# YQChen8/SSF-SLAM

Hardware: AMD Instinct MI355X
Metric: LiDAR front-end frames/sec (mask+feature+GN), 64-beam 120k pts, 1/2/4/8 GPUs (higher is better)
Workload: dtype f32 features / f64 mask+solve

## Files before the change

### ssf-slam_amd/csrc/mask_pose.hip

```cpp
#include "ssf_device.hpp"
#include "ssf_internal.hpp"
#include "svd3.hpp"

#include <float.h>
#include <type_traits>

namespace ssf {

#ifndef SSF_MASK_THREADS
#define SSF_MASK_THREADS 768
#endif
constexpr int kMaskThreads = SSF_MASK_THREADS;

#ifdef SSF_MASK_STAMPS
#define SSF_STAMP(slot)                                                                   \
    do {                                                                                  \
        if (threadIdx.x == 0) {                                                           \
            const unsigned long long _t = __builtin_amdgcn_s_memtime();                   \
            out[26 + (slot)] = (double)(_t - stamp0);                                     \
        }                                                                                 \
    } while (0)
#else
#define SSF_STAMP(slot) do { } while (0)
#endif
constexpr int kNW = kMaskThreads / 64;
#ifndef SSF_LLOYD_DEEP
#define SSF_LLOYD_DEEP 2
#endif
constexpr int kLloydDeep = SSF_LLOYD_DEEP;
#ifndef SSF_KPP_DEEP
#define SSF_KPP_DEEP 2
#endif
constexpr int kKppBlocks = 4096;
constexpr double kPi = 3.14159265358979323846;
#ifndef SSF_LLOYD_FULL_PASSES
#define SSF_LLOYD_FULL_PASSES 4
#endif
constexpr int kLloydFullPasses = SSF_LLOYD_FULL_PASSES;
#ifndef SSF_LLOYD_REFULL
#define SSF_LLOYD_REFULL 4
#endif
constexpr int kLloydRefull = SSF_LLOYD_REFULL;
#ifndef SSF_LLOYD_REC_DEEP
#define SSF_LLOYD_REC_DEEP 8
#endif
constexpr int kLloydRecDeep = SSF_LLOYD_REC_DEEP;
constexpr int kLQ = SSF_LLOYD_REC_DEEP * 128;
constexpr int kLloydMax = 300;

SSF_DEV constexpr int up(int i, int j) { return i * 6 - (i * (i - 1)) / 2 + (j - i); }

struct MaskShared {
    double mean[6], tol;
    double tot[28];
    double cen[12], csn[2], cenp[12], csnp[2];
    double x0[6], ktot[16];
    double mu[12], U[42], logdet[2], logw[2];
    double Aq[21], bq[6], cq, C0;
    double rand1, rand2;
    double lb;
    double C[36], L[36], Li[36];
    double sums[29];
    double lsum[14];
    double lhist[kLloydMax * 9];
    float lb1[512], lb2[512];
    int64_t c0, c1;
    double dg_cyc, dg_n, dg_lab, dg_wfull, dg_full1;
#ifdef SSF_MASK_STAMPS
    double dg_e[3];
#endif
    double passes;
    int km_iter, em_iter, strict, converged, done, status, label0, bg, bg_pred, lfull;
    double hnk[2], hq[2], hpm[12];
    int hrc[2];
};

template <class T>
SSF_DEV void load_x(const T* __restrict__ P, const T* __restrict__ Fl, int64_t i, double x[6]) {
    x[0] = (double)Fl[3 * i]; x[1] = (double)Fl[3 * i + 1]; x[2] = (double)Fl[3 * i + 2];
    x[3] = (double)P[3 * i];  x[4] = (double)P[3 * i + 1];  x[5] = (double)P[3 * i + 2];
}



SSF_DEV int prec_chol6_r(const double (&C)[36], double (&U)[21], double& logdet) {
    double L[36], Li[36];
#pragma unroll
    for (int k = 0; k < 36; ++k) { L[k] = 0.0; Li[k] = 0.0; }
    bool ok = true;
#pragma unroll
    for (int j = 0; j < 6; ++j) {
        double s = C[j * 6 + j];
#pragma unroll
        for (int k = 0; k < j; ++k) s -= L[j * 6 + k] * L[j * 6 + k];
        ok = ok && (s > 0.0);
        L[j * 6 + j] = sqrt(s);
#pragma unroll
        for (int i = j + 1; i < 6; ++i) {
            double v = C[i * 6 + j];
#pragma unroll
            for (int k = 0; k < j; ++k) v -= L[i * 6 + k] * L[j * 6 + k];
            L[i * 6 + j] = v / L[j * 6 + j];
        }
    }
#pragma unroll
    for (int c = 0; c < 6; ++c)
#pragma unroll
        for (int i = c; i < 6; ++i) {
            double v = (i == c) ? 1.0 : 0.0;
#pragma unroll
            for (int k = c; k < i; ++k) v -= L[i * 6 + k] * Li[k * 6 + c];
            Li[i * 6 + c] = v / L[i * 6 + i];
        }
    double ld = 0.0;
#pragma unroll
    for (int i = 0; i < 6; ++i)
#pragma unroll
        for (int j = i; j < 6; ++j) U[up(i, j)] = Li[j * 6 + i];
#pragma unroll
    for (int i = 0; i < 6; ++i) ld += log(Li[i * 6 + i]);
    logdet = ld;
    return ok ? 0 : -1;
}

__device__ __noinline__ int gmm_params2(MaskShared& S, const double* comp1, int init, int64_t n) {
    const int k = (int)(threadIdx.x & 1u);
    const double eps10 = 10.0 * DBL_EPSILON;
    double a[28];
#pragma unroll
    for (int i = 0; i < 28; ++i) a[i] = k == 1 ? comp1[i] : S.tot[i] - comp1[i];
    const double nk = a[0] + eps10;
    double d[6];
#pragma unroll
    for (int i = 0; i < 6; ++i) {
        const double mu = (a[0] * S.mean[i] + a[1 + i]) / nk;
        d[i] = mu - S.mean[i];
        S.hpm[6 * k + i] = mu;
    }
    double C[36];
#pragma unroll
    for (int i = 0; i < 6; ++i)
#pragma unroll
        for (int j = i; j < 6; ++j) {
            double v = a[7 + up(i, j)] - a[1 + i] * d[j] - d[i] * a[1 + j] + a[0] * d[i] * d[j];
            v = v / nk;
            C[i * 6 + j] = v; C[j * 6 + i] = v;
        }
#pragma unroll
    for (int i = 0; i < 6; ++i) C[i * 6 + i] += 1e-6;
    double U[21], ld;
    const int rc = prec_chol6_r(C, U, ld);
    double P[36];
#pragma unroll
    for (int r = 0; r < 6; ++r)
#pragma unroll
        for (int c = r; c < 6; ++c) {
            double v = 0.0;
#pragma unroll
            for (int j = c; j < 6; ++j) v += U[up(r, j)] * U[up(c, j)];
            P[r * 6 + c] = v; P[c * 6 + r] = v;
        }
    double q = 0.0, Pm[6];
#pragma unroll
    for (int r = 0; r < 6; ++r) {
        double v = 0.0;
#pragma unroll
        for (int c = 0; c < 6; ++c) v += P[r * 6 + c] * d[c];
        Pm[r] = v;
        q += d[r] * v;
    }
    S.hnk[k] = nk; S.hq[k] = q; S.hrc[k] = rc;
    __builtin_amdgcn_wave_barrier();
    const bool ok = S.hrc[0] == 0 && S.hrc[1] == 0;
    if (ok) {
#pragma unroll
        for (int i = 0; i < 6; ++i) S.mu[6 * k + i] = S.hpm[6 * k + i];
#pragma unroll
        for (int i = 0; i < 21; ++i) S.U[21 * k + i] = U[i];
        S.logdet[k] = ld;
        double* Pk = k ? S.L : S.C;
#pragma unroll
        for (int i = 0; i < 36; ++i) Pk[i] = P[i];
#pragma unroll
        for (int i = 0; i < 6; ++i) S.hpm[6 * k + i] = Pm[i];
    }
    __builtin_amdgcn_wave_barrier();
    if (k != 0) return 0;
    if (!ok) return -1;
    const double nk0 = S.hnk[0], nk1 = S.hnk[1];
    double w0, w1;
    if (init) { w0 = nk0 / (double)n; w1 = nk1 / (double)n; }
    else { const double sw = nk0 + nk1; w0 = nk0 / sw; w1 = nk1 / sw; }
    S.logw[0] = log(w0); S.logw[1] = log(w1);
    const double* P0 = S.C;
    const double* P1 = S.L;
#pragma unroll
    for (int r = 0; r < 6; ++r) {
#pragma unroll
        for (int c = r; c < 6; ++c) {
            const double A = -0.5 * (P1[r * 6 + c] - P0[r * 6 + c]);
            S.Aq[up(r, c)] = r == c ? A : 2.0 * A;
        }
        S.bq[r] = S.hpm[6 + r] - S.hpm[r];
    }
    S.cq = -0.5 * (S.hq[1] - S.hq[0]) + (S.logdet[1] + S.logw[1]) - (S.logdet[0] + S.logw[0]);
    const double N = S.tot[0];
    double tr = 0.0, lin = 0.0;
#pragma unroll
    for (int r = 0; r < 6; ++r) {
// ... 199 lines not shown
                tt = 1 - m[0][0] + m[1][1] - m[2][2];
                w = m[2][0] - m[0][2]; x = m[0][1] + m[1][0]; y = tt; z = m[1][2] + m[2][1];
            }
        } else {
            if (m[0][0] < -m[1][1]) {
                tt = 1 - m[0][0] - m[1][1] + m[2][2];
                w = m[0][1] - m[1][0]; x = m[2][0] + m[0][2]; y = m[1][2] + m[2][1]; z = tt;
            } else {
                tt = 1 + m[0][0] + m[1][1] + m[2][2];
                w = tt; x = m[1][2] - m[2][1]; y = m[2][0] - m[0][2]; z = m[0][1] - m[1][0];
            }
        }
        const double f = 0.5 / sqrt(tt);
        q[0] = x * f; q[1] = y * f; q[2] = z * f; q[3] = w * f;
    } else if (status == 0) {
        status = SSF_POSE_NOT_ORTHOGONAL;
    }
    for (int i = 0; i < 3; ++i) out[SSF_POSE_OUT_T + i] = t[i];
    for (int i = 0; i < 4; ++i) out[SSF_POSE_OUT_Q + i] = q[i];
    for (int i = 0; i < 9; ++i) out[SSF_POSE_OUT_R + i] = R[i];
    out[SSF_POSE_OUT_NBG] = n;
    return status;
}

constexpr int kSlot = 32;
constexpr int kMaxSplit = kMaskMaxSplit;
constexpr uint32_t kSpinLimit = 1u << 24;
constexpr int kMaxExchanges = 1 + 3 + 300 + 1 + 100 + 1;

struct Split {
    int G, g;
    int64_t r0, r1;
    double* part;
    uint32_t* arrive;
    uint32_t* fail;
    uint32_t seq;
};


SSF_DEV bool wait_arrivals(const Split& X, uint32_t target) {
    uint32_t spins = 0;
    while (__hip_atomic_load(X.arrive, __ATOMIC_RELAXED, __HIP_MEMORY_SCOPE_AGENT) < target) {
        __builtin_amdgcn_s_sleep(2);
        if (++spins > kSpinLimit ||
            __hip_atomic_load(X.fail, __ATOMIC_RELAXED, __HIP_MEMORY_SCOPE_AGENT) != 0u)
            return false;
    }
    return true;
}

template <int N, bool kMin = false>
SSF_DEV bool exchange(Split& X, double (&v)[N], double* tmp, int* okflag) {
    static_assert(N <= kSlot, "exchange: N <= kSlot");
    if (X.G == 1) return true;
    if (X.seq >= (uint32_t)kMaxExchanges) return false;
    double* slot = X.part + (size_t)X.seq * (size_t)X.G * kSlot;
#pragma unroll
    for (int k = 0; k < N; ++k)
        if (threadIdx.x == (unsigned)k)
            __hip_atomic_store(reinterpret_cast<unsigned long long*>(slot + X.g * kSlot + k),
                               (unsigned long long)__double_as_longlong(v[k]), __ATOMIC_RELAXED,
                               __HIP_MEMORY_SCOPE_AGENT);
    X.seq += 1u;
    if (threadIdx.x < 64) {
        asm volatile("s_waitcnt vmcnt(0)" ::: "memory");
        if (threadIdx.x == 0) {
            __builtin_amdgcn_fence(__ATOMIC_RELEASE, "agent");
            asm volatile("s_waitcnt vmcnt(0)" ::: "memory");
            __hip_atomic_fetch_add(X.arrive, 1u, __ATOMIC_RELAXED, __HIP_MEMORY_SCOPE_AGENT);
            const int ok = wait_arrivals(X, (uint32_t)X.G * X.seq) ? 1 : 0;
            __builtin_amdgcn_fence(__ATOMIC_ACQUIRE, "agent");
            asm volatile("s_waitcnt vmcnt(0)" ::: "memory");
            *okflag = ok;
        }
    }
    __syncthreads();
    __builtin_amdgcn_fence(__ATOMIC_ACQUIRE, "wavefront");
    if (!*okflag) return false;
    for (int t = threadIdx.x; t < X.G * N; t += blockDim.x) {
        const int gg = t / N, k = t - gg * N;
        tmp[kSlot + t] = __longlong_as_double((long long)__hip_atomic_load(
            reinterpret_cast<unsigned long long*>(slot + gg * kSlot + k), __ATOMIC_RELAXED,
            __HIP_MEMORY_SCOPE_AGENT));
    }
    __syncthreads();
    if (threadIdx.x < (unsigned)N) {
        double acc = kMin ? __builtin_inf() : 0.0;
        for (int gg = 0; gg < X.G; ++gg) {
            const double x = tmp[kSlot + gg * N + threadIdx.x];
            acc = kMin ? (x < acc ? x : acc) : acc + x;
        }
        tmp[threadIdx.x] = acc;
    }
    __syncthreads();
#pragma unroll
    for (int k = 0; k < N; ++k) v[k] = tmp[k];
    __syncthreads();
    return true;
}

SSF_DEV bool exchange_prefix(Split& X, double v, double* tmp, int* okflag, double& before, double& total) {
    if (X.seq >= (uint32_t)kMaxExchanges) return false;
    double* slot = X.part + (size_t)X.seq * (size_t)X.G * kSlot;
    if (threadIdx.x == 0)
        __hip_atomic_store(reinterpret_cast<unsigned long long*>(slot + X.g * kSlot),
                           (unsigned long long)__double_as_longlong(v), __ATOMIC_RELAXED, __HIP_MEMORY_SCOPE_AGENT);
    X.seq += 1u;
    if (threadIdx.x < 64) {
        asm volatile("s_waitcnt vmcnt(0)" ::: "memory");
        if (threadIdx.x == 0) {
            __builtin_amdgcn_fence(__ATOMIC_RELEASE, "agent");
            asm volatile("s_waitcnt vmcnt(0)" ::: "memory");
            __hip_atomic_fetch_add(X.arrive, 1u, __ATOMIC_RELAXED, __HIP_MEMORY_SCOPE_AGENT);
            const int ok = wait_arrivals(X, (uint32_t)X.G * X.seq) ? 1 : 0;
            __builtin_amdgcn_fence(__ATOMIC_ACQUIRE, "agent");
            asm volatile("s_waitcnt vmcnt(0)" ::: "memory");
            *okflag = ok;
        }
    }
    __syncthreads();
    __builtin_amdgcn_fence(__ATOMIC_ACQUIRE, "wavefront");
    if (!*okflag) return false;
    if (threadIdx.x < (unsigned)X.G)
        tmp[kSlot + threadIdx.x] = __longlong_as_double((long long)__hip_atomic_load(
            reinterpret_cast<unsigned long long*>(slot + threadIdx.x * kSlot), __ATOMIC_RELAXED,
            __HIP_MEMORY_SCOPE_AGENT));
    __syncthreads();
    if (threadIdx.x == 0) {
        double b = 0.0, t = 0.0;
        for (int gg = 0; gg < X.G; ++gg) {
            const double x = tmp[kSlot + gg];
            if (gg < X.g) b += x;
            t += x;
        }
        tmp[0] = b; tmp[1] = t;
    }
    __syncthreads();
    before = tmp[0];
    total = tmp[1];
    __syncthreads();
    return true;
}

SSF_DEV void accum_kabsch(double (&k)[16], const double* x, const double cs[3], const double cd[3]) {
    double s[3], d[3];
    for (int i = 0; i < 3; ++i) { d[i] = x[3 + i] - cd[i]; s[i] = (x[3 + i] + x[i]) - cs[i]; }
    k[0] += 1.0;
#pragma unroll
    for (int i = 0; i < 3; ++i) { k[1 + i] += s[i]; k[4 + i] += d[i]; }
#pragma unroll
    for (int r = 0; r < 3; ++r)
#pragma unroll
        for (int c = 0; c < 3; ++c) k[7 + r * 3 + c] += s[r] * d[c];
}

template <class T>
__global__ __launch_bounds__(kMaskThreads) void k_mask_pose(
    const T* __restrict__ pts, const T* __restrict__ flow,
    const int64_t* __restrict__ frame_off, int mode, const uint8_t* __restrict__ mask_in,
    const double* __restrict__ draws, uint2* __restrict__ lloyd_rec, int reflection,
    uint8_t* __restrict__ bg_mask, double* __restrict__ out_all, int n_frames, int G,
    uint32_t* __restrict__ sync, double* __restrict__ parts, const int32_t* __restrict__ order,
    int tickets) {
    __shared__ MaskShared S;
    __shared__ double red[kNW * 32];
    __shared__ int ired[kNW];
    __shared__ unsigned long long cand_lds[2];
    __shared__ double bsum[kKppBlocks];
    __shared__ uint32_t lq[kNW * kLQ];
    __shared__ double xtmp[kSlot + kMaxSplit * kSlot];
    __shared__ int tk, okflag;
    const int tid = threadIdx.x;
    for (int iter = 0;; ++iter) {
    int f, g = 0;
    if (G == 1 && !tickets) {
        if (iter > 0) break;
        f = blockIdx.x;
    } else {
        __syncthreads();
        if (tid == 0) tk = (int)atomicAdd(sync, 1u);
        __syncthreads();
        f = tk / G;
        g = tk - f * G;
        if (f >= n_frames) break;
    }
    if (order) {
        f = order[f];
        if ((unsigned)f >= (unsigned)n_frames) continue;
    }
    [&]() {
    const int64_t fb = frame_off[f], n = frame_off[f + 1] - fb;
    const T* P = pts + 3 * fb;
    const T* Fl = flow + 3 * fb;
    double* out = out_all + (int64_t)f * SSF_POSE_OUT_STRIDE;
    Split X;
    X.G = G; X.g = g;
    {
        const int64_t chunk = ((n + G - 1) / G + 127) / 128 * 128;
        X.r0 = min(n, (int64_t)g * chunk);
        X.r1 = min(n, X.r0 + chunk);
    }
    X.part = parts + (size_t)f * kMaxExchanges * (size_t)G * kSlot;
    X.arrive = sync + 4 + f;
    X.fail = sync + 4 + n_frames + f;
    X.seq = 0;
    const int64_t r0 = X.r0, r1 = X.r1;
    auto sync_failed = [&]() {
        if (tid == 0) {
            __hip_atomic_store(X.fail, 1u, __ATOMIC_RELAXED, __HIP_MEMORY_SCOPE_AGENT);
            if (g == 0) {
                for (int i = 0; i < SSF_POSE_OUT_STRIDE; ++i) out[i] = 0.0;
                out[SSF_POSE_OUT_STATUS] = SSF_POSE_SYNC_FAILED;
            }
        }
    };
    if (tid == 0) {
        S.passes = 0; S.status = 0; S.km_iter = 0; S.em_iter = 0; S.converged = 0;
        if (g == 0) for (int i = 26; i < SSF_POSE_OUT_STRIDE; ++i) out[i] = 0.0;
    }
#ifdef SSF_MASK_STAMPS
    const unsigned long long stamp0 = __builtin_amdgcn_s_memtime();
#endif
    __syncthreads();

    if (mode != SSF_MASK_GMM) {
        double cs[3] = {0, 0, 0}, cd[3] = {0, 0, 0};
        if (n > 0) {
            double x0[6];
            load_x(P, Fl, 0, x0);
            for (int i = 0; i < 3; ++i) { cd[i] = x0[3 + i]; cs[i] = x0[3 + i] + x0[i]; }
        }
        double k[16];
        for (int i = 0; i < 16; ++i) k[i] = 0.0;
        for (int64_t i = tid; i < n; i += blockDim.x) {
            const uint8_t mv = mask_in[fb + i];
            const bool bg = (mode == SSF_MASK_GT) ? (mv == 0) : (mv != 0);
            if (bg_mask) bg_mask[fb + i] = bg ? 1 : 0;
            if (!bg) continue;
            double x[6];
            load_x(P, Fl, i, x);
            accum_kabsch(k, x, cs, cd);
        }
        block_sum_rs<16>(k, red);
        if (tid == 0) {
            for (int i = 0; i < SSF_POSE_OUT_STRIDE; ++i) out[i] = 0.0;
            for (int i = 0; i < 16; ++i) S.sums[i] = k[i];
            const int st = kabsch_finish(S.sums, cs, cd, reflection, out);
            out[SSF_POSE_OUT_STATUS] = st;
            out[SSF_POSE_OUT_BGLABEL] = -1;
            out[SSF_POSE_OUT_PASSES] = 1;
        }
        return;
    }

    if (n < 2) {
        if (tid == 0 && g == 0) {
            for (int i = 0; i < SSF_POSE_OUT_STRIDE; ++i) out[i] = 0.0;
            out[SSF_POSE_OUT_STATUS] = SSF_POSE_GMM_FAILED;
        }
        return;
    }

    {
        double x0[6];
        load_x(P, Fl, 0, x0);
        double a[27];
#pragma unroll
        for (int i = 0; i < 27; ++i) a[i] = 0.0;
        for_points_deep<kLloydDeep>(P, Fl, r0, r1, [&](int64_t, const double* x, bool val) {
            double v[6], vw[6];
#pragma unroll
            for (int d = 0; d < 6; ++d) { v[d] = x[d] - x0[d]; vw[d] = val ? v[d] : 0.0; a[d] += vw[d]; }
#pragma unroll
            for (int r = 0; r < 6; ++r)
#pragma unroll
                for (int c = r; c < 6; ++c) a[6 + up(r, c)] += vw[r] * v[c];
        });
        block_sum_rs<27>(a, red);
        if (!exchange<27>(X, a, xtmp, &okflag)) { sync_failed(); return; }
        if (tid == 0) {
            const double nn = (double)n;
            double m[6];
            double tol = 0.0;
            for (int d = 0; d < 6; ++d) { m[d] = a[d] / nn; S.mean[d] = x0[d] + m[d]; }
            S.tot[0] = nn;
            for (int d = 0; d < 6; ++d) S.tot[1 + d] = a[d] - nn * m[d];
            for (int r = 0; r < 6; ++r)
                for (int c = r; c < 6; ++c) S.tot[7 + up(r, c)] = a[6 + up(r, c)] - nn * m[r] * m[c];
            for (int d = 0; d < 6; ++d) tol += S.tot[7 + up(d, d)] / nn;
            S.tol = tol / 6.0 * 1e-4;
            for (int d = 0; d < 6; ++d) S.x0[d] = x0[d];
            S.ktot[0] = nn;
            for (int r = 0; r < 3; ++r) { S.ktot[1 + r] = a[r] + a[3 + r]; S.ktot[4 + r] = a[3 + r]; }
            for (int r = 0; r < 3; ++r)
                for (int c = 0; c < 3; ++c) {
                    const int fr = r, pr = 3 + r, pc = 3 + c;
                    const double sfp = a[6 + (fr <= pc ? up(fr, pc) : up(pc, fr))];
                    const double spp = a[6 + (pr <= pc ? up(pr, pc) : up(pc, pr))];
                    S.ktot[7 + r * 3 + c] = sfp + spp;
                }
            S.c0 = (int64_t)draws[3 * f];
            if (S.c0 < 0) S.c0 = 0;
            if (S.c0 >= n) S.c0 = n - 1;
            S.passes = 1;
        }
        __syncthreads();
    }
    SSF_STAMP(0);
    double mean[6];
#pragma unroll
    for (int d = 0; d < 6; ++d) mean[d] = uni(S.mean[d]);

    {
        double c0[6], cn0 = 0.0;
        {
            double x[6];
            load_x(P, Fl, S.c0, x);
            for (int d = 0; d < 6; ++d) { c0[d] = x[d] - mean[d]; cn0 += c0[d] * c0[d]; }
        }
        const int nw = blockDim.x >> 6, w = tid >> 6, lane = lane_id();
        const int64_t nloc = r1 - r0;
        const int64_t seg = (((nloc + nw - 1) / nw) + 63) / 64 * 64;
        const int64_t ws = r0 + (int64_t)w * seg, we = ws + seg < r1 ? ws + seg : r1;
        auto dist0x = [&](const double* x) {
            double dt = 0.0, xs = 0.0;
#pragma unroll
            for (int d = 0; d < 6; ++d) { const double v = x[d] - mean[d]; dt += c0[d] * v; xs += v * v; }
            const double v = (-2.0 * dt + cn0) + xs;
            return v > 0.0 ? v : 0.0;
        };
        auto dist0 = [&](int64_t i) {
            double x[6];
            load_x(P, Fl, i, x);
            return dist0x(x);
        };
        constexpr int kKppDeep = SSF_KPP_DEEP;
        const int64_t wlast = we > ws ? we - 1 : ws;
        const int64_t spw = seg / 64;
        const bool use_blocks = spw * nw <= kKppBlocks;
        double wsum = 0.0;
        T kb[kKppDeep][6];
        if (ws < we) {
#pragma unroll
            for (int k = 0; k < kKppDeep; ++k) load_raw(P, Fl, min(ws + 64 * k + lane, wlast), kb[k]);
        }
        for (int64_t b0 = ws; b0 < we; b0 += 64 * kKppDeep)
#pragma unroll
        for (int k = 0; k < kKppDeep; ++k) {
            const int64_t b = b0 + 64 * k;
            if (b >= we) break;
            const int64_t i = b + lane;
            double x[6];
#pragma unroll
            for (int d = 0; d < 6; ++d) x[d] = (double)kb[k][d];
            load_raw(P, Fl, min(i + 64 * kKppDeep, wlast), kb[k]);
            const double d = i < we ? dist0x(x) : 0.0;
            wsum += d;
            if (use_blocks) {
                double v = d;
#pragma unroll
                for (int o = 1; o < 64; o <<= 1) {
                    const double y = __shfl_up(v, o, 64);
                    if (lane >= o) v += y;
                }
                if (lane == 63) bsum[w * spw + (b - ws) / 64] = v;
            }
        }
        wsum = wave_sum(wsum);
        if (lane == 0) red[w] = wsum;
        if (tid == 0) { cand_lds[0] = (unsigned long long)n; cand_lds[1] = (unsigned long long)n; }
        __syncthreads();
        double pot = 0.0, carry = 0.0;
        for (int k = 0; k < nw; ++k) { if (k == w) carry = pot; pot += red[k]; }
        if (G > 1) {
            double before = 0.0, total = 0.0;
            if (!exchange_prefix(X, pot, xtmp, &okflag, before, total)) { sync_failed(); return; }
            carry += before;
            pot = total;
        }
        if (tid == 0) {
            S.rand1 = draws[3 * f + 1] * pot;
            S.rand2 = draws[3 * f + 2] * pot;
            S.passes += 1;
        }
        const double r1 = draws[3 * f + 1] * pot, r2 = draws[3 * f + 2] * pot;
        const double wtot = red[w];
        bool f1 = carry + wtot < r1 * (1.0 - 1e-9), f2 = carry + wtot < r2 * (1.0 - 1e-9);
        if (use_blocks) {
            int64_t blk1 = -1, blk2 = -1;
            double cb1 = 0.0, cb2 = 0.0;
            if (lane == 0 && !(f1 && f2)) {
                double cr = carry;
                for (int64_t k = 0; ws + 64 * k < we; ++k) {
                    const double tot = bsum[w * spw + k];
                    if (!f1 && blk1 < 0 && cr + tot >= r1) { blk1 = k; cb1 = cr; }
                    if (!f2 && blk2 < 0 && cr + tot >= r2) { blk2 = k; cb2 = cr; }
                    if ((f1 || blk1 >= 0) && (f2 || blk2 >= 0)) break;
                    cr += tot;
                }
            }
            blk1 = __shfl(blk1, 0, 64); blk2 = __shfl(blk2, 0, 64);
            cb1 = __shfl(cb1, 0, 64); cb2 = __shfl(cb2, 0, 64);
#pragma unroll
            for (int j = 0; j < 2; ++j) {
                const int64_t blk = j ? blk2 : blk1;
                if (blk < 0) continue;
                const int64_t b = ws + 64 * blk;
                const int64_t i = b + lane;
                double v = i < we ? dist0(i) : 0.0;
#pragma unroll
                for (int o = 1; o < 64; o <<= 1) {
                    const double y = __shfl_up(v, o, 64);
                    if (lane >= o) v += y;
                }
                const double incl = (j ? cb2 : cb1) + v;
                const uint64_t mm = __ballot(i < we && incl >= (j ? r2 : r1));
                if (mm && lane == 0) atomicMin(&cand_lds[j], (unsigned long long)(b + __ffsll((unsigned long long)mm) - 1));
            }
            f1 = f2 = true;
        }
        for (int64_t b = ws; b < we && !(f1 && f2); b += 64) {
            const int64_t i = b + lane;
            double v = i < we ? dist0(i) : 0.0;
#pragma unroll
            for (int o = 1; o < 64; o <<= 1) {
                const double y = __shfl_up(v, o, 64);
                if (lane >= o) v += y;
            }
            const double incl = carry + v;
            const uint64_t m1 = __ballot(i < we && incl >= r1), m2 = __ballot(i < we && incl >= r2);
            if (!f1 && m1) { f1 = true; if (lane == 0) atomicMin(&cand_lds[0], (unsigned long long)(b + __ffsll((unsigned long long)m1) - 1)); }
            if (!f2 && m2) { f2 = true; if (lane == 0) atomicMin(&cand_lds[1], (unsigned long long)(b + __ffsll((unsigned long long)m2) - 1)); }
            carry += __shfl(v, 63, 64);
        }
        __syncthreads();
        double cmin[2] = {(double)cand_lds[0], (double)cand_lds[1]};
        if (!exchange<2, true>(X, cmin, xtmp, &okflag)) { sync_failed(); return; }
        const int64_t cand[2] = {cmin[0] < (double)n ? (int64_t)cmin[0] : n - 1,
                                 cmin[1] < (double)n ? (int64_t)cmin[1] : n - 1};
        double cc[2][6], ccn[2] = {0.0, 0.0};
        for (int j = 0; j < 2; ++j) {
            double x[6];
            load_x(P, Fl, cand[j], x);
            for (int d = 0; d < 6; ++d) { cc[j][d] = x[d] - mean[d]; ccn[j] += cc[j][d] * cc[j][d]; }
        }
        double cp[2] = {0.0, 0.0};
        if (ws < we) {
#pragma unroll
            for (int k = 0; k < kKppDeep; ++k) load_raw(P, Fl, min(ws + 64 * k + lane, wlast), kb[k]);
        }
        for (int64_t b0 = ws; b0 < we; b0 += 64 * kKppDeep)
#pragma unroll
        for (int k = 0; k < kKppDeep; ++k) {
            const int64_t b = b0 + 64 * k;
            if (b >= we) break;
            const int64_t i = b + lane;
            double x[6];
#pragma unroll
            for (int d = 0; d < 6; ++d) x[d] = (double)kb[k][d];
            load_raw(P, Fl, min(i + 64 * kKppDeep, wlast), kb[k]);
            if (i < we) {
                double xs = 0.0, dt0 = 0.0, dt1 = 0.0, dtc = 0.0;
#pragma unroll
                for (int d = 0; d < 6; ++d) {
                    const double v = x[d] - mean[d];
                    dtc += c0[d] * v; xs += v * v; dt0 += cc[0][d] * v; dt1 += cc[1][d] * v;
                }
                double di = (-2.0 * dtc + cn0) + xs;
                di = di > 0.0 ? di : 0.0;
                double v0 = (-2.0 * dt0 + ccn[0]) + xs, v1 = (-2.0 * dt1 + ccn[1]) + xs;
                v0 = v0 > 0.0 ? v0 : 0.0; v1 = v1 > 0.0 ? v1 : 0.0;
                cp[0] += v0 < di ? v0 : di;
                cp[1] += v1 < di ? v1 : di;
            }
        }
        block_sum<2>(cp, red);
        if (!exchange<2>(X, cp, xtmp, &okflag)) { sync_failed(); return; }
        if (tid == 0) {
            const int best = cp[1] < cp[0] ? 1 : 0;
            S.c1 = cand[best];
            for (int d = 0; d < 6; ++d) { S.cen[d] = c0[d]; S.cen[6 + d] = cc[best][d]; }
            for (int d = 0; d < 12; ++d) S.cenp[d] = 0.0;
            S.csnp[0] = S.csnp[1] = 0.0;
            S.passes += 2;
        }
        __syncthreads();
    }

    SSF_STAMP(1);
    if (tid == 0) { S.strict = 0; S.done = 0; S.lfull = 1; S.dg_cyc = S.dg_n = S.dg_lab = S.dg_wfull = S.dg_full1 = 0.0; }
    uint2* __restrict__ LR = lloyd_rec + ((fb + 2 * (int64_t)f + 1) & ~(int64_t)1);
    uint32_t* __restrict__ LQ =
        reinterpret_cast<uint32_t*>(lloyd_rec + frame_off[n_frames] + 2 * (int64_t)n_frames + 2) + fb +
        64 * (int64_t)f;
    for (int it = 0; it < kLloydMax; ++it) {
        if (tid == 0) {
            double* h = S.lhist + 9 * it;
            for (int k = 0; k < 2; ++k) {
                double sn = 0.0;
                for (int d = 0; d < 6; ++d) sn += S.cen[6 * k + d] * S.cen[6 * k + d];
                S.csn[k] = sn;
            }
            for (int d = 0; d < 6; ++d) h[d] = S.cen[6 + d] - S.cen[d];
            h[6] = S.csn[0] - S.csn[1];
            h[7] = sqrt(S.csn[0]) + sqrt(S.csn[1]);
            h[8] = S.csn[0] + S.csn[1];
        }
        __syncthreads();
        if (tid < it) {
            const double* h = S.lhist + 9 * it;
            const double* g = S.lhist + 9 * tid;
            double dw = 0.0;
            for (int d = 0; d < 6; ++d) dw += (h[d] - g[d]) * (h[d] - g[d]);
            S.lb1[tid] = __double2float_ru(2.0 * sqrt(dw) + 2e-13 * (h[7] + g[7]));
            S.lb2[tid] = __double2float_ru(fabs(h[6] - g[6]) + 1e-13 * (h[8] + g[8]));
        }
        __syncthreads();
        const double csn0 = uni(S.csn[0]), csn1 = uni(S.csn[1]);
        double acc[14];
#pragma unroll
        for (int k = 0; k < 14; ++k) acc[k] = 0.0;
        int changed = 0, nlab = 0;
        const bool full = S.lfull != 0;
#ifdef SSF_MASK_STAMPS
        const unsigned long long pass_t0 = __builtin_amdgcn_s_memtime();
#endif
        const bool wrec = it >= kLloydFullPasses - 1;
        auto label = [&](auto wrec_c, int64_t i, const double* x, int lp, bool val) {
            const LdsDouble* cen = lds_laundered(S.cen);
            double v[6], dt0 = 0.0, dt1 = 0.0, vn = 0.0;
#pragma unroll
            for (int d = 0; d < 6; ++d) {
                v[d] = x[d] - mean[d];
                dt0 += v[d] * cen[d]; dt1 += v[d] * cen[6 + d]; vn += v[d] * v[d];
            }
            const double D0 = -2.0 * dt0 + csn0, D1 = -2.0 * dt1 + csn1;
            const int l = D1 < D0 ? 1 : 0;
            double d1 = full ? (double)l : (double)(l - lp), d0 = full ? 1.0 - d1 : -d1;
            d1 = val ? d1 : 0.0; d0 = val ? d0 : 0.0;
            changed += val && (it == 0 || l != lp);
            acc[0] += d0; acc[7] += d1;
#pragma unroll
            for (int d = 0; d < 6; ++d) { acc[1 + d] += d0 * v[d]; acc[8 + d] += d1 * v[d]; }
            const uint32_t gb = __float_as_uint((float)fabs(D0 - D1));
            const uint32_t nvb = (__float_as_uint(__builtin_sqrtf((float)vn)) + 4u + 0x1FFu) & 0x7FFFFE00u;
            if constexpr (decltype(wrec_c)::value) LR[val ? i : n] = make_uint2(gb ? gb - 1u : 0u, nvb | (uint32_t)it | ((uint32_t)l << 31));
        };
        if (full) {
            const double cpn0 = uni(S.csnp[0]), cpn1 = uni(S.csnp[1]);
            auto full_pass = [&](auto wrec_c) {
                for_points_deep<kLloydDeep>(P, Fl, r0, r1, [&](int64_t i, const double* x, bool val) {
                    const LdsDouble* cenp = lds_laundered(S.cenp);
                    double dp0 = 0.0, dp1 = 0.0;
#pragma unroll
                    for (int d = 0; d < 6; ++d) {
                        const double v = x[d] - mean[d];
                        dp0 += v * cenp[d]; dp1 += v * cenp[6 + d];
                    }
                    const int lp = (-2.0 * dp1 + cpn1) < (-2.0 * dp0 + cpn0) ? 1 : 0;
                    label(wrec_c, i, x, lp, val);
                });
            };
            if (wrec) full_pass(std::true_type{});
            else full_pass(std::false_type{});
            nlab = (int)((r1 - r0 - tid + blockDim.x - 1) / blockDim.x);
        } else {
            const int w = __builtin_amdgcn_readfirstlane(tid >> 6), lane = lane_id();
            const int64_t seg = ((r1 - r0 + kNW - 1) / kNW + 127) / 128 * 128;
            const int64_t ws = r0 + (int64_t)w * seg, we = ws + seg < r1 ? ws + seg : r1;
            uint32_t* __restrict__ WQ = LQ + ws;
            const int64_t qspare = n - ws;
            const uint4* __restrict__ LR4 = reinterpret_cast<const uint4*>(LR);
            const int64_t plast = (n - 1) >> 1;
            uint32_t* Q = lq + w * kLQ;
            int qc = 0, nl = 0;
            constexpr int D = kLloydRecDeep;
            uint4 buf[D];
#pragma unroll
            for (int d = 0; d < D; ++d) buf[d] = LR4[min((ws >> 1) + d * 64 + lane, plast)];
            for (int64_t base = ws; base < we; base += D * 128) {
#pragma unroll
                for (int d = 0; d < D; ++d) {
                    const int64_t b = base + d * 128;
                    const uint4 q = buf[d];
#pragma unroll
                    for (int h = 0; h < 2; ++h) {
                        const uint32_t gx = h ? q.z : q.x, gy = h ? q.w : q.y;
                        const int64_t i = b + 2 * lane + h;
                        const int tr = (int)(gy & 0x1FFu);
                        const float nv = __uint_as_float(gy & 0x7FFFFE00u);
                        const bool skip = __uint_as_float(gx) > __builtin_fmaf(S.lb1[tr], nv, S.lb2[tr]) * 1.00001f;
                        const bool nd = (i < we) & !skip;
                        const uint64_t m = __ballot(nd);
                        if (nd) Q[nl + __popcll(m & lanemask_lt())] = (uint32_t)i | (gy & 0x80000000u);
                        nl += __popcll(m);
                    }
                    buf[d] = LR4[min(((b + D * 128) >> 1) + lane, plast)];
                }
                __builtin_amdgcn_wave_barrier();
#pragma unroll
                for (int h = 0; h < 2; ++h)
                    WQ[h * 64 + lane < nl ? qc + h * 64 + lane : qspare + lane] = Q[h * 64 + lane];
                for (int k = 128; k < nl; k += 64)
                    if (k + lane < nl) WQ[qc + k + lane] = Q[k + lane];
                __builtin_amdgcn_wave_barrier();
                qc += nl;
                nl = 0;
            }
            __threadfence_block();
            for (int j0 = 0; j0 < qc; j0 += 512) {
                uint32_t e[8];
#pragma unroll
                for (int k = 0; k < 8; ++k) e[k] = WQ[min(j0 + k * 64 + lane, qc - 1)];
                T px[8][6];
#pragma unroll
                for (int k = 0; k < 8; ++k) load_raw(P, Fl, (int64_t)(e[k] & 0x7FFFFFFFu), px[k]);
#pragma unroll
                for (int k = 0; k < 8; ++k) {
                    double x[6];
#pragma unroll
                    for (int d = 0; d < 6; ++d) x[d] = (double)px[k][d];
                    const bool val = j0 + k * 64 + lane < qc;
                    label(std::true_type{}, (int64_t)(e[k] & 0x7FFFFFFFu), x, (int)(e[k] >> 31), val);
                    nlab += val ? 1 : 0;
                }
            }
        }
        block_sum_rs<14>(acc, red);
        changed = block_sum_scalar<int>(changed, ired);
        nlab = block_sum_scalar<int>(nlab, ired);
        if (G > 1) {
            double v[16];
#pragma unroll
            for (int k = 0; k < 14; ++k) v[k] = acc[k];
            v[14] = (double)changed; v[15] = (double)nlab;
            if (!exchange<16>(X, v, xtmp, &okflag)) { sync_failed(); return; }
#pragma unroll
            for (int k = 0; k < 14; ++k) acc[k] = v[k];
            changed = (int)v[14]; nlab = (int)v[15];
        }
        if (tid == 0) {
            S.passes += full ? 1.0 + (wrec ? 8.0 / 24.0 : 0.0)
                             : (8.0 * (double)n + 40.0 * (double)nlab) / (24.0 * (double)n);
            S.km_iter = it + 1;
            for (int k = 0; k < 14; ++k) S.lsum[k] = full ? acc[k] : S.lsum[k] + acc[k];
            S.lfull = full ? it < kLloydFullPasses - 1 : nlab * kLloydRefull > n;
#ifdef SSF_MASK_STAMPS
            if (!full) { S.dg_cyc += (double)(__builtin_amdgcn_s_memtime() - pass_t0); S.dg_n += 1.0; S.dg_lab += nlab; }
            else if (it == kLloydFullPasses - 1) S.dg_wfull = (double)(__builtin_amdgcn_s_memtime() - pass_t0);
            else if (it == 1) S.dg_full1 = (double)(__builtin_amdgcn_s_memtime() - pass_t0);
#endif
            for (int k = 0; k < 12; ++k) S.cenp[k] = S.cen[k];
            S.csnp[0] = S.csn[0]; S.csnp[1] = S.csn[1];
            double shift = 0.0;
            for (int k = 0; k < 2; ++k) {
                const double wgt = S.lsum[7 * k];
                double sh = 0.0;
                for (int d = 0; d < 6; ++d) {
                    const double nc = wgt > 0.0 ? S.lsum[7 * k + 1 + d] * (1.0 / wgt) : S.cen[6 * k + d];
                    const double df = nc - S.cen[6 * k + d];
                    sh += df * df;
                    S.cen[6 * k + d] = nc;
                }
                sh = sqrt(sh);
                shift += sh * sh;
            }
            if (changed == 0) { S.strict = 1; S.done = 1; }
            else if (shift <= S.tol) S.done = 1;
        }
        __syncthreads();
        if (S.done) break;
    }

    SSF_STAMP(2);
    {
        double cen[12], csn0, csn1;
        if (S.strict) {
#pragma unroll
            for (int k = 0; k < 12; ++k) cen[k] = uni(S.cenp[k]);
            csn0 = S.csnp[0]; csn1 = S.csnp[1];
        } else {
#pragma unroll
            for (int k = 0; k < 12; ++k) cen[k] = uni(S.cen[k]);
            csn0 = 0.0; csn1 = 0.0;
            for (int d = 0; d < 6; ++d) { csn0 += cen[d] * cen[d]; csn1 += cen[6 + d] * cen[6 + d]; }
        }
        double acc[28];
#pragma unroll
        for (int k = 0; k < 28; ++k) acc[k] = 0.0;
        for_points_deep<kLloydDeep>(P, Fl, r0, r1, [&](int64_t, const double* x, bool val) {
            double v[6], dt0 = 0.0, dt1 = 0.0;
#pragma unroll
            for (int d = 0; d < 6; ++d) { v[d] = x[d] - mean[d]; dt0 += v[d] * cen[d]; dt1 += v[d] * cen[6 + d]; }
            const int l = (-2.0 * dt1 + csn1) < (-2.0 * dt0 + csn0) ? 1 : 0;
            const double w1 = val ? (double)l : 0.0;
            acc[0] += w1;
#pragma unroll
            for (int a = 0; a < 6; ++a) {
                const double wv = w1 * v[a];
                acc[1 + a] += wv;
#pragma unroll
                for (int b = a; b < 6; ++b) acc[7 + up(a, b)] += wv * v[b];
            }
        });
        block_sum_rs<28>(acc, red);
        if (!exchange<28>(X, acc, xtmp, &okflag)) { sync_failed(); return; }
        if (tid < 2) {
            if (tid == 0) {
                S.passes += 1;
                for (int k = 0; k < 28; ++k) S.sums[k] = acc[k];
            }
            const int rc = gmm_params2(S, S.sums, 1, n);
            if (tid == 0) {
                if (rc != 0) S.status = SSF_POSE_GMM_FAILED;
                S.lb = -__builtin_inf();
                S.done = 0;
            }
        }
        __syncthreads();
    }

    SSF_STAMP(3);
    for (int it = 1; it <= 100 && S.status == 0; ++it) {
        const double cq = uni(S.cq);
        double acc[29];
#pragma unroll
        for (int k = 0; k < 29; ++k) acc[k] = 0.0;
        double prod = 1.0;
        int pexp = 0;
#ifdef SSF_MASK_STAMPS
        if (it == 1 && tid == 0) S.dg_e[0] = S.dg_e[1] = S.dg_e[2] = 0.0;
        const unsigned long long e_t0 = __builtin_amdgcn_s_memtime();
#endif
        const LdsDouble* AqL = lds_laundered(S.Aq);
        const LdsDouble* bqL = lds_laundered(S.bq);
        auto em_point = [&](const double* v, double dl) {
            const double e = exp(-fabs(dl));
            const double d = 1.0 + e;
            acc[28] += dl > 0.0 ? dl : 0.0;
            const double inv = recip_1_2(d);
            const double r = dl > 0.0 ? inv : e * inv;
            acc[0] += r;
#pragma unroll
            for (int a = 0; a < 6; ++a) {
                const double rv = r * v[a];
                acc[1 + a] += rv;
#pragma unroll
                for (int b = a; b < 6; ++b) acc[7 + up(a, b)] += rv * v[b];
            }
            return d;
        };
        auto renorm = [&]() {
            pexp += __builtin_amdgcn_frexp_exp(prod);
            prod = __builtin_amdgcn_frexp_mant(prod);
        };
        for_point_pairs(P, Fl, r0, r1, [&](const double* xa, const double* xb) {
            double va[6], vb[6];
#pragma unroll
            for (int a = 0; a < 6; ++a) { va[a] = xa[a] - mean[a]; vb[a] = xb[a] - mean[a]; }
            double da, db;
            asm volatile("" ::: "memory");
            em_delta2(va, vb, AqL, bqL, cq, da, db);
            prod *= em_point(va, da);
            prod *= em_point(vb, db);
            renorm();
        }, [&](const double* xa) {
            double va[6];
#pragma unroll
            for (int a = 0; a < 6; ++a) va[a] = xa[a] - mean[a];
            prod *= em_point(va, em_delta1(va, AqL, bqL, cq));
            renorm();
        });
        acc[28] += log(prod) + (double)pexp * 0.69314718055994530942;
        block_sum_rs<29>(acc, red);
#ifdef SSF_MASK_STAMPS
        const unsigned long long e_t1 = __builtin_amdgcn_s_memtime();
#endif
        if (!exchange<29>(X, acc, xtmp, &okflag)) { sync_failed(); return; }
#ifdef SSF_MASK_STAMPS
        const unsigned long long e_t2 = __builtin_amdgcn_s_memtime();
#endif
        if (tid < 2) {
            double prev = 0.0;
            if (tid == 0) {
                S.passes += 1;
                S.em_iter = it;
                prev = S.lb;
                S.lb = (S.C0 + acc[28]) / (double)n;
                for (int k = 0; k < 29; ++k) S.sums[k] = acc[k];
            }
            const int rc = gmm_params2(S, S.sums, 0, n);
            if (tid == 0) {
                if (rc != 0) S.status = SSF_POSE_GMM_FAILED;
                if (fabs(S.lb - prev) < 1e-3) { S.converged = 1; S.done = 1; }
            }
        }
        __syncthreads();
#ifdef SSF_MASK_STAMPS
        if (tid == 0) {
            S.dg_e[0] += (double)(e_t1 - e_t0); S.dg_e[1] += (double)(e_t2 - e_t1);
            S.dg_e[2] += (double)(__builtin_amdgcn_s_memtime() - e_t2);
        }
#endif
        if (S.done) break;
    }

    SSF_STAMP(4);
    {
        const int pred = S.logw[1] > S.logw[0] ? 1 : 0;
        const double cq = uni(S.cq);
        double x0[6];
#pragma unroll
        for (int d = 0; d < 6; ++d) x0[d] = uni(S.x0[d]);
        double k1[16];
#pragma unroll
        for (int i = 0; i < 16; ++i) k1[i] = 0.0;
        if (tid == 0) S.label0 = 0;
        __syncthreads();
        for_points_deep<kLloydDeep>(P, Fl, r0, r1, [&](int64_t i, const double* x, bool val) {
            const LdsDouble* Aq = lds_laundered(S.Aq);
            const LdsDouble* bq = lds_laundered(S.bq);
// ... 151 lines not shown
```

Baseline: 61710.

## Fuse first Lloyd assignment pass into k-means++ candidate scoring pass

The k-means++ second-seed scoring pass now also accumulates the per-cluster label sums for both candidate seeds. The first Lloyd iteration is then finished from those sums after the best candidate is chosen, so the loop starts at iteration 1 and one full pass over the points is saved. In exchange the kpp pass carries 28 extra accumulators, does a wider block reduction and a 30-value cross-GPU exchange. The shared epilogue was moved into a noinline helper. The skipped iteration's pass cost is no longer added to the passes counter, and register pressure rises in the kpp loop.

```diff
diff --git a/ssf-slam_amd/csrc/mask_pose.hip b/ssf-slam_amd/csrc/mask_pose.hip
--- a/ssf-slam_amd/csrc/mask_pose.hip
+++ b/ssf-slam_amd/csrc/mask_pose.hip
@@ -55,6 +55,7 @@
     double tot[28];
     double cen[12], csn[2], cenp[12], csnp[2];
     double x0[6], ktot[16];
+    double kpp[21];
     double mu[12], U[42], logdet[2], logw[2];
     double Aq[21], bq[6], cq, C0;
     double rand1, rand2;
@@ -560,6 +561,39 @@
     for (int r = 0; r < 3; ++r)
 #pragma unroll
         for (int c = 0; c < 3; ++c) k[7 + r * 3 + c] += s[r] * d[c];
+}
+
+SSF_DEV void lloyd_history(MaskShared& S, int it) {
+    double* h = S.lhist + 9 * it;
+    for (int d = 0; d < 6; ++d) h[d] = S.cen[6 + d] - S.cen[d];
+    h[6] = S.csn[0] - S.csn[1];
+    h[7] = sqrt(S.csn[0]) + sqrt(S.csn[1]);
+    h[8] = S.csn[0] + S.csn[1];
+}
+
+__device__ __noinline__ void lloyd_epilogue(MaskShared& S, int it, bool full, double cost, bool any_changed,
+                                            int nlab, int64_t n) {
+    S.passes += cost;
+    S.km_iter = it + 1;
+    for (int k = 0; k < 14; ++k) S.lsum[k] = full ? S.sums[k] : S.lsum[k] + S.sums[k];
+    S.lfull = full ? it < kLloydFullPasses - 1 : nlab * kLloydRefull > n;
+    for (int k = 0; k < 12; ++k) S.cenp[k] = S.cen[k];
+    S.csnp[0] = S.csn[0]; S.csnp[1] = S.csn[1];
+    double shift = 0.0;
+    for (int k = 0; k < 2; ++k) {
+        const double wgt = S.lsum[7 * k];
+        double sh = 0.0;
+        for (int d = 0; d < 6; ++d) {
+            const double nc = wgt > 0.0 ? S.lsum[7 * k + 1 + d] * (1.0 / wgt) : S.cen[6 * k + d];
+            const double df = nc - S.cen[6 * k + d];
+            sh += df * df;
+            S.cen[6 * k + d] = nc;
+        }
+        sh = sqrt(sh);
+        shift += sh * sh;
+    }
+    if (!any_changed) { S.strict = 1; S.done = 1; }
+    else if (shift <= S.tol) S.done = 1;
 }
 
 template <class T>
@@ -852,7 +886,15 @@
             load_x(P, Fl, cand[j], x);
             for (int d = 0; d < 6; ++d) { cc[j][d] = x[d] - mean[d]; ccn[j] += cc[j][d] * cc[j][d]; }
         }
+        if (tid == 0) {
+            for (int d = 0; d < 6; ++d) { S.kpp[d] = c0[d]; S.kpp[6 + d] = cc[0][d]; S.kpp[12 + d] = cc[1][d]; }
+            S.kpp[18] = cn0; S.kpp[19] = ccn[0]; S.kpp[20] = ccn[1];
+        }
+        __syncthreads();
         double cp[2] = {0.0, 0.0};
+        double la[28];
+#pragma unroll
+        for (int k = 0; k < 28; ++k) la[k] = 0.0;
         if (ws < we) {
 #pragma unroll
             for (int k = 0; k < kKppDeep; ++k) load_raw(P, Fl, min(ws + 64 * k + lane, wlast), kb[k]);
@@ -868,51 +910,65 @@
             for (int d = 0; d < 6; ++d) x[d] = (double)kb[k][d];
             load_raw(P, Fl, min(i + 64 * kKppDeep, wlast), kb[k]);
             if (i < we) {
-                double xs = 0.0, dt0 = 0.0, dt1 = 0.0, dtc = 0.0;
+                const LdsDouble* kp = lds_laundered(S.kpp);
+                double v[6], xs = 0.0, dt[2] = {0.0, 0.0}, dtc = 0.0;
 #pragma unroll
                 for (int d = 0; d < 6; ++d) {
-                    const double v = x[d] - mean[d];
-                    dtc += c0[d] * v; xs += v * v; dt0 += cc[0][d] * v; dt1 += cc[1][d] * v;
+                    v[d] = x[d] - mean[d];
+                    dtc += kp[d] * v[d]; xs += v[d] * v[d]; dt[0] += kp[6 + d] * v[d]; dt[1] += kp[12 + d] * v[d];
                 }
-                double di = (-2.0 * dtc + cn0) + xs;
+                const double D0 = -2.0 * dtc + kp[18];
+                double di = D0 + xs;
                 di = di > 0.0 ? di : 0.0;
-                double v0 = (-2.0 * dt0 + ccn[0]) + xs, v1 = (-2.0 * dt1 + ccn[1]) + xs;
-                v0 = v0 > 0.0 ? v0 : 0.0; v1 = v1 > 0.0 ? v1 : 0.0;
-                cp[0] += v0 < di ? v0 : di;
-                cp[1] += v1 < di ? v1 : di;
+#pragma unroll
+                for (int j = 0; j < 2; ++j) {
+                    const double D1 = -2.0 * dt[j] + kp[19 + j];
+                    double vj = D1 + xs;
+                    vj = vj > 0.0 ? vj : 0.0;
+                    cp[j] += vj < di ? vj : di;
+                    const double d1 = D1 < D0 ? 1.0 : 0.0, d0 = 1.0 - d1;
+                    la[14 * j] += d0; la[14 * j + 7] += d1;
+#pragma unroll
+                    for (int d = 0; d < 6; ++d) { la[14 * j + 1 + d] += d0 * v[d]; la[14 * j + 8 + d] += d1 * v[d]; }
+                }
             }
         }
         block_sum<2>(cp, red);
-        if (!exchange<2>(X, cp, xtmp, &okflag)) { sync_failed(); return; }
+        block_sum_rs<28>(la, red);
+        double pl[30];
+        pl[0] = cp[0]; pl[1] = cp[1];
+#pragma unroll
+        for (int k = 0; k < 28; ++k) pl[2 + k] = la[k];
+        if (!exchange<30>(X, pl, xtmp, &okflag)) { sync_failed(); return; }
         if (tid == 0) {
-            const int best = cp[1] < cp[0] ? 1 : 0;
+            const int best = pl[1] < pl[0] ? 1 : 0;
             S.c1 = cand[best];
-            for (int d = 0; d < 6; ++d) { S.cen[d] = c0[d]; S.cen[6 + d] = cc[best][d]; }
-            for (int d = 0; d < 12; ++d) S.cenp[d] = 0.0;
-            S.csnp[0] = S.csnp[1] = 0.0;
+            for (int d = 0; d < 6; ++d) { S.cen[d] = S.kpp[d]; S.cen[6 + d] = S.kpp[6 + 6 * best + d]; }
             S.passes += 2;
+            S.strict = 0; S.done = 0; S.lfull = 1;
+            S.dg_cyc = S.dg_n = S.dg_lab = S.dg_wfull = S.dg_full1 = 0.0;
+            S.csn[0] = S.kpp[18]; S.csn[1] = S.kpp[19 + best];
+            lloyd_history(S, 0);
+            for (int k = 0; k < 14; ++k) S.sums[k] = pl[2 + 14 * best + k];
+            lloyd_epilogue(S, 0, true, 0.0, true, (int)n, n);
         }
         __syncthreads();
     }
 
     SSF_STAMP(1);
-    if (tid == 0) { S.strict = 0; S.done = 0; S.lfull = 1; S.dg_cyc = S.dg_n = S.dg_lab = S.dg_wfull = S.dg_full1 = 0.0; }
     uint2* __restrict__ LR = lloyd_rec + ((fb + 2 * (int64_t)f + 1) & ~(int64_t)1);
     uint32_t* __restrict__ LQ =
         reinterpret_cast<uint32_t*>(lloyd_rec + frame_off[n_frames] + 2 * (int64_t)n_frames + 2) + fb +
         64 * (int64_t)f;
-    for (int it = 0; it < kLloydMax; ++it) {
+    if (!S.done)
+    for (int it = 1; it < kLloydMax; ++it) {
         if (tid == 0) {
-            double* h = S.lhist + 9 * it;
             for (int k = 0; k < 2; ++k) {
                 double sn = 0.0;
                 for (int d = 0; d < 6; ++d) sn += S.cen[6 * k + d] * S.cen[6 * k + d];
                 S.csn[k] = sn;
             }
-            for (int d = 0; d < 6; ++d) h[d] = S.cen[6 + d] - S.cen[d];
-            h[6] = S.csn[0] - S.csn[1];
-            h[7] = sqrt(S.csn[0]) + sqrt(S.csn[1]);
-            h[8] = S.csn[0] + S.csn[1];
+            lloyd_history(S, it);
         }
         __syncthreads();
         if (tid < it) {
@@ -946,7 +1002,7 @@
             const int l = D1 < D0 ? 1 : 0;
             double d1 = full ? (double)l : (double)(l - lp), d0 = full ? 1.0 - d1 : -d1;
             d1 = val ? d1 : 0.0; d0 = val ? d0 : 0.0;
-            changed += val && (it == 0 || l != lp);
+            changed += val && l != lp;
             acc[0] += d0; acc[7] += d1;
 #pragma unroll
             for (int d = 0; d < 6; ++d) { acc[1 + d] += d0 * v[d]; acc[8 + d] += d1 * v[d]; }
@@ -1048,33 +1104,15 @@
             changed = (int)v[14]; nlab = (int)v[15];
         }
         if (tid == 0) {
-            S.passes += full ? 1.0 + (wrec ? 8.0 / 24.0 : 0.0)
-                             : (8.0 * (double)n + 40.0 * (double)nlab) / (24.0 * (double)n);
-            S.km_iter = it + 1;
-            for (int k = 0; k < 14; ++k) S.lsum[k] = full ? acc[k] : S.lsum[k] + acc[k];
-            S.lfull = full ? it < kLloydFullPasses - 1 : nlab * kLloydRefull > n;
+            const double cost = full ? 1.0 + (wrec ? 8.0 / 24.0 : 0.0)
+                                     : (8.0 * (double)n + 40.0 * (double)nlab) / (24.0 * (double)n);
 #ifdef SSF_MASK_STAMPS
             if (!full) { S.dg_cyc += (double)(__builtin_amdgcn_s_memtime() - pass_t0); S.dg_n += 1.0; S.dg_lab += nlab; }
             else if (it == kLloydFullPasses - 1) S.dg_wfull = (double)(__builtin_amdgcn_s_memtime() - pass_t0);
             else if (it == 1) S.dg_full1 = (double)(__builtin_amdgcn_s_memtime() - pass_t0);
 #endif
-            for (int k = 0; k < 12; ++k) S.cenp[k] = S.cen[k];
-            S.csnp[0] = S.csn[0]; S.csnp[1] = S.csn[1];
-            double shift = 0.0;
-            for (int k = 0; k < 2; ++k) {
-                const double wgt = S.lsum[7 * k];
-                double sh = 0.0;
-                for (int d = 0; d < 6; ++d) {
-                    const double nc = wgt > 0.0 ? S.lsum[7 * k + 1 + d] * (1.0 / wgt) : S.cen[6 * k + d];
-                    const double df = nc - S.cen[6 * k + d];
-                    sh += df * df;
-                    S.cen[6 * k + d] = nc;
-                }
-                sh = sqrt(sh);
-                shift += sh * sh;
-            }
-            if (changed == 0) { S.strict = 1; S.done = 1; }
-            else if (shift <= S.tol) S.done = 1;
+            for (int k = 0; k < 14; ++k) S.sums[k] = acc[k];
+            lloyd_epilogue(S, it, full, cost, changed != 0, nlab, n);
         }
         __syncthreads();
         if (S.done) break;
```

Result: no change. 62110 (median of 6 runs) (+0.6%).
